# WilliamYi96/HGR-Net

Measured on AMD Instinct MI355X. Metric: images/sec over 21K-class hierarchy, batch 512; hit@1 parity vs reference, higher is better.
Workload: dtype f16

## Files before the change

hgr-net_amd/_lib.py:

```python
from __future__ import annotations

import ctypes as C
import os
from pathlib import Path

import torch

_HERE = Path(__file__).resolve().parent
LIB_PATH = Path(os.environ.get("HGR_LIB", _HERE / "lib" / "libhgr.so"))

HGR_BF16, HGR_F16 = 0, 1
EPI_NONE, EPI_BIAS, EPI_BIAS_QUICKGELU, EPI_BIAS_RESIDUAL, EPI_BIAS_RELU, EPI_BIAS_ADD16_RELU, EPI_ACCUM, EPI_QGELU_GRAD16 = 0, 1, 2, 3, 4, 5, 6, 7

_p, _i, _l, _f = C.c_void_p, C.c_int, C.c_int64, C.c_float

SIGNATURES = {
    "hgr_gemm_nt": [_p, _l, _p, _l, _p, _l, _p, _p, _l, _i, _i, _i, _i, _i, _i, _p],
    "hgr_gemm_set_tile": [_i],
    "hgr_gemm_set_tail": [_i, _i],
    "hgr_gemm_set_persist": [_i],
    "hgr_gemm_set_ws": [_i],
    "hgr_gemm_set_p8": [_i],
    "hgr_im2col_patches": [_p, _p, _i, _i, _i, _i, _i, _p],
    "hgr_im2col_patches_ex": [_p, _p, _i, _i, _i, _i, _i, _i, _i, _p],
# ... 41 lines not shown
    "hgr_ctx_splice_bwd": [_p, _p, _i, _i, _i, _i, _p],
    "hgr_sumsq": [_p, _l, _p, _p],
    "hgr_eval_counters": [_p, _i, _p, _i, _p, _p, _i, _p, _p, _i, _p, _i, _p],
    "hgr_eval_counters_rows": [_p, _i, _p, _p, _p, _i, _p, _p, _p, _i, _p, _i, _p],
    "hgr_eval_report_rows": [_p, _i, _p, _p, _p, _i, _p, _p, _p, _i, _p, _i, _p],
    "hgr_path_scores": [_p, _l, _p, _l, _i, _p, _p, _p, _i, _p],
    "hgr_subtree_hedge": [_p, _l, _i, _p, _p, _p, _f, _p, _i, _p, _p, _p, _l, _i, _p],
    "hgr_hedge_counters_rows": [_p, _i, _p, _p, _p, _i, _p, _i, _p],
    "hgr_set_ranks": [_p, _l, _i, _p, _p, _i, _p, _p, _p, _i, _p],
    "hgr_set_counters_rows": [_p, _p, _i, _p, _p, _i, _p, _p, _p, _i, _p, _i, _p],
    "hgr_dot_f32":[_p, _p, _l, _p, _f, _i, _p],
    "hgr_conv3x3_nhwc_plain": [_p, _p, _p, _i, _i, _i, _i, _i, _i, _i, _p],
    "hgr_gemm_nt_splitk": [_p, _l, _p, _l, _p, _l, _i, _i, _i, _i, _i, _p],
    "hgr_gemm_tn_splitk": [_p, _l, _p, _l, _p, _l, _i, _i, _i, _i, _i, _p],
    "hgr_gemm_tn_tile": [_i, _i],
    "hgr_gemm_plan_capture": [_p, _i],
    "hgr_conv3x3_wgrad_splitk": [_p, _l, _p, _p, _l, _i, _i, _i, _i, _i, _i, _i, _p],
    "hgr_relu_bwd16": [_p, _p, _p, _l, _i, _p],
    "hgr_add16": [_p, _p, _p, _l, _i, _p],
    "hgr_avgpool2_bwd_nhwc": [_p, _p, _i, _i, _i, _i, _i, _p],
    "hgr_attnpool_tokens_bwd": [_p, _p, _i, _i, _i, _i, _p],
    "hgr_im2col3x3_t": [_p, _p, _i, _i, _i, _i, _l, _i, _p],
    "hgr_bn_fold": [_p, _p, _p, _p, _p, _f, _p, _p, _i, _i, _i, _i, _i, _p],
    "hgr_bn_unfold_grad": [_p, _l, _p, _p, _p, _p, _p, _f, _p, _p, _p, _i, _i, _i, _p],
    "hgr_csr_group_aggregate": [_p, _l, _p, _p, _p, _p, _i, _p, _p, _p, _p, _i, _p, _p, _p, _p, _i, _p, _p, _l, _i, _f, _i, _p],
    "hgr_gemm_nt_res_stats": [_p, _l, _p, _l, _p, _p, _l, _p, _p, _i, _i, _i, _i, _p],
    "hgr_vit_head": [_p, _p, _l, _l, _p, _p, _f, _p, _p, _i, _i, _i, _i, _p],
    "hgr_gemm_nt_res_stats_guard": [_p, _l, _p, _l, _p, _p, _l, _p, _p, _f, _p, _i, _i, _i, _i, _p],
    "hgr_gemm_nt_ln": [_p, _l, _p, _l, _p, _l, _p, _p, _p, _f, _i, _i, _i, _i, _i, _p],
    "hgr_gemm_nt_ln_mha": [_p, _l, _p, _l, _p, _p, _p, _f, _p, _l, _i, _i, _i, _i, _i, _p],
    "hgr_gemm_nt_bias_gelu_dual": [_p, _l, _p, _l, _p, _l, _p, _l, _p, _i, _i, _i, _i, _p],
    "hgr_gemm_nt_qgelu_grad_colsum": [_p, _l, _p, _l, _p, _l, _p, _l, _p, _i, _i, _i, _i, _p],
    "hgr_vit_embed_ln_stats": [_p, _p, _p, _p, _p, _p, _p, _p, _i, _i, _i, _f, _i, _p],
    "hgr_row_stats16": [_p, _p, _p, _p, _i, _i, _i, _p],
    "hgr_pair_rows_f32": [_p, _p, _p, _i, _i, _l, _p, _i, _p],
    "hgr_logits_eval_workspace_bytes": [_i, _i],
    "hgr_logits_eval": [_p, _p, _i, _i, _i, _p, _p, _p, _i, _p, _p, _i, _p, _i, _i, _p, _p, _p, _p, _i, _p],
    "hgr_logits_eval_tile_stage": [_p, _p, _i, _i, _i, _p, _p, _p, _i, _p, _p, _i, _p, _i, _i, _p, _p, _p, _p, _i, _p],
    "hgr_logits_eval_row_stage": [_p, _p, _i, _i, _i, _p, _p, _p, _i, _p, _p, _i, _p, _i, _i, _p, _p, _p, _p, _i, _p],
    "hgr_comm_unique_id": [_p],
    "hgr_comm_init": [_i, _i, _p],
    "hgr_comm_destroy": [],
    "hgr_comm_rank": [],
    "hgr_comm_world": [],
    "hgr_allreduce": [_p, _p, _l, _i, _i, _p],
    "hgr_allgather": [_p, _p, _l, _i, _p],
    "hgr_broadcast": [_p, _l, _i, _i, _p],
    "hgr_adamw": [_p, _p, _p, _p, _l, _f, _f, _f, _f, _f, _i, _p, _f, _f, _p],
}


class GemmLaunch(C.Structure):
    _fields_ = [(name, C.c_int32) for name in ("kernel", "variant", "epilogue", "out_f32", "act", "grid_x", "grid_y", "tiles_m", "tiles_n", "total",
                                                "nbig", "big_panels", "tiles_m_half", "group", "m_fastest", "vec_ok", "row0", "rows")]


class HgrError(RuntimeError):
    pass


_lib = None


ABI_VERSION = 5


# ... 43 lines not shown
```

hgr-net_amd/clip/model.py:

```python
from __future__ import annotations

import os
from collections import OrderedDict
from typing import Dict, Optional, Tuple, Union

import numpy as np
import torch
from torch import nn

from .. import ops
from .._lib import (EPI_BIAS, EPI_BIAS_ADD16_RELU, EPI_BIAS_QUICKGELU, EPI_BIAS_RELU, EPI_BIAS_RESIDUAL, EPI_NONE,
                    HgrError)


class QuickGELU(nn.Module):
    """Placeholder so ``mlp`` keeps the reference's child names (c_fc, gelu, c_proj); the activation
    itself is fused into the c_fc GEMM epilogue (HGR_EPI_BIAS_QUICKGELU)."""


class ResidualAttentionBlock(nn.Module):
    def __init__(self, d_model: int, n_head: int):
        super().__init__()
        self.attn = nn.MultiheadAttention(d_model, n_head)
        self.ln_1 = nn.LayerNorm(d_model)
# ... 99 lines not shown
        w32, g32, be32 = w.detach().float(), ln.weight.detach().float(), ln.bias.detach().float()
        wf = (w32 * g32[None, :]).to(dt).contiguous()
        return wf, wf.float().sum(dim=1).contiguous(), (w32 @ be32 + b.detach().float()).contiguous()


class _Workspace:

    def __init__(self):
        self._b: Dict[str, torch.Tensor] = {}
        self.epoch = 0

    def const(self, name: str, build) -> torch.Tensor:
        t = self._b.get("const." + name)
        if t is None:
            t = self._b["const." + name] = build()
            self.epoch += 1
        return t

    def get(self, name: str, shape, dtype, device) -> torch.Tensor:
        n = int(np.prod(shape))
        t = self._b.get(name)
        if t is None or t.numel() < n or t.dtype != dtype or t.device != device:
            t = torch.empty(n, dtype=dtype, device=device)
            self._b[name] = t
            self.epoch += 1
        return t[:n].view(*shape)


IMG_STREAMS = max(1, int(os.environ.get("HGR_IMG_STREAMS", "1")))
IMG_STREAMS_MIN_ROWS = 8192
CLS_LAST = os.environ.get("HGR_CLS_LAST", "1") != "0"
LN_FUSED = os.environ.get("HGR_LN_FUSED", "1") != "0"
QKV_MHA = os.environ.get("HGR_QKV_MHA", "1") != "0"


def ln_fusable(w: int, m: int = 0) -> bool:
    return LN_FUSED and w % 128 == 0 and m * 4 * w * 2 < 2 ** 32


def _run_blocks(x: Optional[torch.Tensor], blocks, heads: int, b: int, l: int, causal: bool, dt: torch.dtype, ws: _Workspace, tag: str,
                taps: Optional[dict] = None, tap_prefix: str = "", pair=None, stats: Optional[torch.Tensor] = None,
                flag: Optional[torch.Tensor] = None, cls_only_last: bool = False):
    m, w = (pair[0] if pair is not None else x).shape
    dev = (pair[0] if pair is not None else x).device
    qkv = ws.get(tag + ".qkv", (m, 3 * w), dt, dev)
    att = ws.get(tag + ".att", (m, w), dt, dev)
    u16 = ws.get(tag + ".u16", (m, 4 * w), dt, dev)
    if pair is not None:
        xh, xl = pair
        for i, k in enumerate(blocks):
            last_cls = cls_only_last and i == len(blocks) - 1 and l > 1 and 3 * w * l < (1 << 23)
            fused_attn = QKV_MHA and not last_cls and ops.ln_mha_ok(w, l, m, xh.stride(0))
            if last_cls:
                ch, cl = xh.view(b, l, w)[:, 0, :], xl.view(b, l, w)[:, 0, :]
                ops.gemm_nt_ln(xh, k.wf_in[w:], qkv[:, w:], k.s_in[w:], k.c_in[w:], stats, k.eps1, tag="kv")
                ops.split_point("class_token_tail")
                st_q = ws.get(tag + ".stats_q", (b, w // 64, 2), torch.float32, dev)
                idx = ws.const(f"cls_rows.{b}.{l}", lambda: (torch.arange(b, dtype=torch.int32, device=dev) * l).contiguous())
                ops.rows_gather(stats.view(b * l, -1), idx, st_q.view(b, -1))
                ops.gemm_nt_ln(ch, k.wf_in[:w], qkv.view(b, l, 3 * w)[:, 0, :w], k.s_in[:w], k.c_in[:w], st_q, k.eps1, tag="q_cls")
            elif fused_attn:
                ops.gemm_nt_ln_mha(xh, k.wf_in, att, k.s_in, k.c_in, stats, b, l, heads, causal, k.eps1)
            else:
                ops.gemm_nt_ln(xh, k.wf_in, qkv, k.s_in, k.c_in, stats, k.eps1, tag="qkv")
            if not fused_attn:
                ops.mha(qkv, att, b, l, heads, causal, q_rows=1 if last_cls else 0)
# ... 285 lines not shown
            fused = self._vit_forward(image, p, out, tag, taps, u8)
            if fused and self._ln_check("v", dev):
                self._vit_forward(image, p, out, tag, taps, u8)
            return out
        main = torch.cuda.current_stream()
        side = self._side_streams(ns - 1, dev)
        cut = [b * i // ns for i in range(ns + 1)]
        fused = False
        for i in range(ns):
            st = main if i == 0 else side[i - 1]
            if i:
                st.wait_stream(main)
            with torch.cuda.stream(st):
                fused |= self._vit_forward(image[cut[i]:cut[i + 1]], p, out[cut[i]:cut[i + 1]], f"v{i}" if i else "v", None, u8)
        for st in side:
            main.wait_stream(st)
        if fused and self._ln_check("v", dev):
            self._vit_forward(image, p, out, "v", None, u8)
        return out

    def _side_streams(self, n: int, dev):
        have = self.__dict__.setdefault("_streams", [])
        while len(have) < n:
            have.append(torch.cuda.Stream(device=dev))
        return have[:n]

    def _vit_forward(self, image: torch.Tensor, p: dict, out: torch.Tensor, tag: str, taps: Optional[dict], u8: bool) -> bool:
        v = self.visual
        dt, ws, dev = self.image_dtype, self._ws, image.device
        b, r = image.shape[0], v.input_resolution
        ps = v.patch_size
        g = r // ps
        gg, l, w = g * g, g * g + 1, v.conv1.weight.shape[0]
        patches = ws.get(tag + ".patches", (b * gg, p["kp"]), dt, dev)
        if u8:
            ops.im2col_patches_u8(image, patches, ps)
        else:
            ops.im2col_patches(image, patches, ps)
        pe = ws.get(tag + ".pe", (b * gg, w), torch.float32, dev)
        ops.gemm_nt(patches, p["conv_w_nhwc"] if u8 else p["conv_w"], pe, tag="patch")
        cls16 = ws.get(tag + ".cls16", (b, w), dt, dev)
        fused = ln_fusable(w, b * l) and "v" not in self._ln_off
        if fused:
            xh = ws.get(tag + ".xh", (b * l, w), dt, dev)
            xl = ws.get(tag + ".xl", (b * l, w), ops.PAIR_LO, dev)
            stats = ws.get(tag + ".stats", (b * l, w // 64, 2), torch.float32, dev)
            ops.vit_embed_ln_stats(pe, p["cls"], p["pos"], p["ln_pre"][0], p["ln_pre"][1], xh, xl, stats, b, gg)
            if taps is not None:
                taps["visual.ln_pre"] = ops.pair_value(xh, xl).view(b, l, w)
            _run_blocks(None, p["vblocks"], w // 64, b, l, False, dt, ws, tag, taps, "visual.transformer", (xh, xl), stats, self._ln_flag("v", dev),
                        cls_only_last=taps is None and CLS_LAST)
            if w <= 1920 and w % 32 == 0 and v.output_dim % 4 == 0:
                ops.vit_head(xh, xl, l, p["ln_post"][0], p["ln_post"][1], float(v.ln_post.eps), p["proj_t"], out)
                return fused
            cls32 = ws.get(tag + ".cls32", (b, w), torch.float32, dev)
            ops.pair_rows_f32(xh, xl, cls32, row_mul=l)
            ops.layernorm(cls32, p["ln_post"][0], p["ln_post"][1], cls16, rows=b)
        else:
            x = ws.get(tag + ".x", (b * l, w), torch.float32, dev)
            ops.vit_embed_ln(pe, p["cls"], p["pos"], p["ln_pre"][0], p["ln_pre"][1], x, b, gg)
            if taps is not None:
                taps["visual.ln_pre"] = x.view(b, l, w).clone()
            _run_blocks(x, p["vblocks"], w // 64, b, l, False, dt, ws, tag, taps, "visual.transformer")
            ops.layernorm(x, p["ln_post"][0], p["ln_post"][1], cls16, rows=b, row_mul=l)
        ops.gemm_nt(cls16, p["proj_t"], out)
        return fused

    @torch.no_grad()
    def encode_text(self, text: torch.Tensor, trim: bool = True, ctx: Optional[torch.Tensor] = None) -> torch.Tensor:
        if not text.is_cuda:
            raise HgrError("encode_text needs a device tensor: the product path has no CPU fallback")
        p = self._prepared()
        dt, ws, dev = self.text_dtype, self._ws, text.device
        text = text.long()
        n, ctx_len = text.shape
        w = self.transformer.width
        d = self.text_projection.shape[1]
        out = torch.empty((n, d), dtype=torch.float32, device=dev)
        eot = torch.empty(n, dtype=torch.int32, device=dev)
        ops.eot_index(text, eot)
# ... 68 lines not shown
```

hgr-net_amd/csrc/hgr_common.h:

```cpp
#pragma once
#include <hip/hip_runtime.h>
#include <stdint.h>
#include <stdio.h>
#include <stdarg.h>
#include <stdlib.h>
#include <type_traits>

#include "../../include/hgr.h"

#define HGR_WAVE 64

#ifdef HGR_LAB
#define HGR_LAB_ON(expr) (expr)
static inline int hgr_lab_env(const char *name) { const char *e = getenv(name); return e ? atoi(e) : 0; }
#else
#define HGR_LAB_ON(expr) false
static inline int hgr_lab_env(const char *) { return 0; }
#endif

typedef __attribute__((ext_vector_type(8))) __bf16 bf16x8;
typedef __attribute__((ext_vector_type(8))) _Float16 f16x8;
typedef __attribute__((ext_vector_type(4))) __bf16 bf16x4;
typedef __attribute__((ext_vector_type(4))) _Float16 f16x4;
typedef __attribute__((ext_vector_type(4))) float f32x4;
// ... 128 lines not shown
__device__ __forceinline__ float wave_max(float v) {
#pragma unroll
    for (int o = 32; o > 0; o >>= 1) v = fmaxf(v, __shfl_xor(v, o));
    return v;
}
__device__ __forceinline__ unsigned long long wave_max_u64(unsigned long long v) {
#pragma unroll
    for (int o = 32; o > 0; o >>= 1) {
        const unsigned lo = __shfl_xor((unsigned)v, o), hi = __shfl_xor((unsigned)(v >> 32), o);
        const unsigned long long w = ((unsigned long long)hi << 32) | lo;
        v = w > v ? w : v;
    }
    return v;
}

__device__ __forceinline__ unsigned orderable(float v) { const unsigned u = __float_as_uint(v); return u ^ ((u >> 31) ? 0xFFFFFFFFu : 0x80000000u); }
__device__ __forceinline__ float unorderable(unsigned u) { return __uint_as_float(u ^ ((u >> 31) ? 0x80000000u : 0xFFFFFFFFu)); }
__device__ __forceinline__ unsigned long long key_of(float v, int p) { return ((unsigned long long)orderable(v) << 32) | (unsigned)(0x7fffffff - p); }
__device__ __forceinline__ void key_decode(unsigned long long m, float &v, int &p) { v = unorderable((unsigned)(m >> 32)); p = 0x7fffffff - (int)(unsigned)m; }

__device__ __forceinline__ int level_pick(const int32_t *__restrict__ lv_row, int n_levels, int le) {
    return (unsigned)le < (unsigned)n_levels ? lv_row[le] : -2;
}
__device__ __forceinline__ unsigned path_edges(unsigned mm, int L) { return L == 1 ? (mm & 1u) : (unsigned)__popc(mm & (mm >> 1)); }

__device__ __forceinline__ float row16_sum(float v) {
    v += __builtin_bit_cast(float, __builtin_amdgcn_update_dpp(0, __builtin_bit_cast(int, v), 0xB1, 0xF, 0xF, true));
    v += __builtin_bit_cast(float, __builtin_amdgcn_update_dpp(0, __builtin_bit_cast(int, v), 0x4E, 0xF, 0xF, true));
    v += __builtin_bit_cast(float, __builtin_amdgcn_update_dpp(0, __builtin_bit_cast(int, v), 0x141, 0xF, 0xF, true));
    v += __builtin_bit_cast(float, __builtin_amdgcn_update_dpp(0, __builtin_bit_cast(int, v), 0x140, 0xF, 0xF, true));
    return v;
}

int hgr_set_error(int code, const char *fmt, ...);

#define HGR_REQUIRE(cond, ...)                                            \
    do {                                                                  \
        if (!(cond)) return hgr_set_error(HGR_EINVAL, __VA_ARGS__);       \
    } while (0)

#define HGR_CHECK_LAUNCH(name)                                                                      \
    do {                                                                                            \
        hipError_t e__ = hipGetLastError();                                                         \
        if (e__ != hipSuccess) return hgr_set_error(HGR_ELAUNCH, "%s: %s", name, hipGetErrorString(e__)); \
    } while (0)

static inline bool hgr_aligned(const void *p, size_t a) { return (reinterpret_cast<uintptr_t>(p) % a) == 0; }

int hgr_cu_count();

template <typename T = int> struct HgrKnob {
    const char *env; T def; T (*clamp)(T) = nullptr;
    bool known = false; T v = T();
    T get() {
        if (!known) {
            const char *e = getenv(env);
            v = !e ? def : std::is_floating_point<T>::value ? (T)atof(e) : (T)atoi(e);
            if (clamp) v = clamp(v);
            known = true;
        }
        return v;
    }
    T set(T nv) { const T prev = get(); v = nv; return prev; }
};
static inline int hgr_knob_bool(int v) { return v != 0; }
```

hgr-net_amd/csrc/hgr_norm.hip:

```cpp
#include "hgr_common.h"

namespace {

constexpr int MAXV = 16;

template <int DT, bool OUT32, int NV>
__global__ __launch_bounds__(256) void layernorm_rows(const float *__restrict__ x, const float *__restrict__ gamma,
                                                      const float *__restrict__ beta, void *__restrict__ y,
                                                      int rows, int W, int64_t row_mul, const int32_t *__restrict__ row_idx, float eps) {
    const int lane = threadIdx.x & 63;
    const int row = blockIdx.x * 4 + (threadIdx.x >> 6);
    if (row >= rows) return;
    const int64_t src = (int64_t)row * row_mul + (row_idx ? row_idx[row] : 0);
    const f32x4 *xr = (const f32x4 *)(x + src * W);
    const int nv = W >> 2;
    f32x4 v[NV];
    float s = 0.f;
#pragma unroll
    for (int i = 0; i < NV; ++i) {
        const int c = i * 64 + lane;
        if (i * 64 < nv) {
            v[i] = (c < nv) ? xr[c] : (f32x4){0.f, 0.f, 0.f, 0.f};
            s += v[i][0] + v[i][1] + v[i][2] + v[i][3];
        }
// ... 18 lines not shown
            f32x4 o;
#pragma unroll
            for (int e = 0; e < 4; ++e) o[e] = (v[i][e] - mean) * rstd * ga[e] + be[e];
            if (OUT32) ((f32x4 *)((float *)y + (int64_t)row * W))[c] = o;
            else ((typename T16<DT>::vec4 *)((typename T16<DT>::elem *)y + (int64_t)row * W))[c] = cvt4<DT>(o[0], o[1], o[2], o[3]);
        }
    }
}

template <int NV, int DT = HGR_F16, bool STATS = false>
__global__ __launch_bounds__(256) void vit_embed_ln(const float *__restrict__ patches, const float *__restrict__ cls,
                                                    const float *__restrict__ pos, const float *__restrict__ gamma,
                                                    const float *__restrict__ beta, float *__restrict__ x,
                                                    int B, int G, int W, float eps, void *__restrict__ xh = nullptr, void *__restrict__ xl = nullptr,
                                                    float *__restrict__ stats = nullptr) {
    const int lane = threadIdx.x & 63;
    const int L = G + 1;
    const int row = blockIdx.x * 4 + (threadIdx.x >> 6);
    if (row >= B * L) return;
    const int b = row / L, t = row - b * L;
    const f32x4 *src = (const f32x4 *)(t == 0 ? cls : patches + ((int64_t)b * G + (t - 1)) * W);
    const f32x4 *pr = (const f32x4 *)(pos + (int64_t)t * W);
    const int nv = W >> 2;
    f32x4 v[NV];
    float s = 0.f;
#pragma unroll
    for (int i = 0; i < NV; ++i) {
        const int c = i * 64 + lane;
        if (i * 64 < nv) {
            v[i] = (c < nv) ? (src[c] + pr[c]) : (f32x4){0.f, 0.f, 0.f, 0.f};
            s += v[i][0] + v[i][1] + v[i][2] + v[i][3];
        }
    }
    const float mean = wave_sum(s) / (float)W;
    float q = 0.f;
#pragma unroll
    for (int i = 0; i < NV; ++i) {
        const int c = i * 64 + lane;
        if (i * 64 < nv && c < nv) {
#pragma unroll
            for (int e = 0; e < 4; ++e) { const float d = v[i][e] - mean; q += d * d; }
        }
    }
    const float rstd = rsqrtf(wave_sum(q) / (float)W + eps);
    const f32x4 *gv = (const f32x4 *)gamma, *bv = (const f32x4 *)beta;
    f32x4 *out = STATS ? nullptr : (f32x4 *)(x + (int64_t)row * W);
#pragma unroll
    for (int i = 0; i < NV; ++i) {
        const int c = i * 64 + lane;
        if (i * 64 < nv && c < nv) {
            const f32x4 ga = gv[c], be = bv[c];
            f32x4 o;
#pragma unroll
            for (int e = 0; e < 4; ++e) o[e] = (v[i][e] - mean) * rstd * ga[e] + be[e];
            if (!STATS) out[c] = o;
            if (STATS) {
                typename T16<DT>::vec4 nh;
                unsigned nl = 0u;
#pragma unroll
                for (int e = 0; e < 4; ++e) { unsigned q; typename T16<DT>::elem h; pair_split<DT>(o[e], h, q); nh[e] = h; nl |= q << (8 * e); }
                ((typename T16<DT>::vec4 *)((typename T16<DT>::elem *)xh + (int64_t)row * W))[c] = nh;
                ((unsigned *)((unsigned char *)xl + (int64_t)row * W))[c] = nl;
                const float s1 = row16_sum((o[0] + o[1]) + (o[2] + o[3]));
                const float s2 = row16_sum((o[0] * o[0] + o[1] * o[1]) + (o[2] * o[2] + o[3] * o[3]));
                if ((lane & 15) == 0) *(float2 *)(stats + ((int64_t)row * (W >> 6) + (c >> 4)) * 2) = make_float2(s1, s2);
            }
        }
    }
}

template <int DT>
__global__ __launch_bounds__(256) void row_stats16(const float *__restrict__ x, void *__restrict__ xh, void *__restrict__ xl, float *__restrict__ stats, int rows, int W) {
    const int lane = threadIdx.x & 63;
    const int row = blockIdx.x * 4 + (threadIdx.x >> 6);
    if (row >= rows) return;
    const f32x4 *xr = (const f32x4 *)(x + (int64_t)row * W);
    const int nv = W >> 2;
    for (int c0 = 0; c0 < nv; c0 += 64) {
        const int c = c0 + lane;
        const bool ok = c < nv;
        const f32x4 v = ok ? xr[c] : (f32x4){0.f, 0.f, 0.f, 0.f};
        const float s1 = row16_sum((v[0] + v[1]) + (v[2] + v[3]));
        const float s2 = row16_sum((v[0] * v[0] + v[1] * v[1]) + (v[2] * v[2] + v[3] * v[3]));
        if (ok) {
            typename T16<DT>::vec4 nh;
            unsigned nl = 0u;
#pragma unroll
            for (int e = 0; e < 4; ++e) { unsigned q; typename T16<DT>::elem h; pair_split<DT>(v[e], h, q); nh[e] = h; nl |= q << (8 * e); }
            ((typename T16<DT>::vec4 *)((typename T16<DT>::elem *)xh + (int64_t)row * W))[c] = nh;
            ((unsigned *)((unsigned char *)xl + (int64_t)row * W))[c] = nl;
            if ((lane & 15) == 0) *(float2 *)(stats + ((int64_t)row * (W >> 6) + (c >> 4)) * 2) = make_float2(s1, s2);
        }
    }
}

template <int DT>
__global__ __launch_bounds__(256) void pair_rows_f32(const void *__restrict__ xh, const void *__restrict__ xl, float *__restrict__ out, int rows, int W,
                                                     int64_t row_mul, const int32_t *__restrict__ row_idx) {
    const int lane = threadIdx.x & 63;
    const int row = blockIdx.x * 4 + (threadIdx.x >> 6);
    if (row >= rows) return;
// ... 253 lines not shown
```

hgr-net_amd/ops.py:

```python
from __future__ import annotations

import math
from typing import Optional

import torch

from . import _lib
from ._lib import (EPI_ACCUM, EPI_BIAS, EPI_BIAS_ADD16_RELU, EPI_BIAS_QUICKGELU, EPI_BIAS_RELU, EPI_BIAS_RESIDUAL, EPI_NONE, EPI_QGELU_GRAD16,
                   HGR_BF16, HGR_F16)

PROFILE = None

WEIGHTS_GEN = [0]

SPLIT_HOOK = None


def split_point(name: str) -> None:
    h = SPLIT_HOOK
    if h is not None:
        h(name)


TORCH16 = {HGR_BF16: torch.bfloat16, HGR_F16: torch.float16}
# ... 114 lines not shown
    assert x16.stride(1) == wfold.stride(1) == out.stride(1) == 1 and stats.dtype == torch.float32 and stats.numel() >= m * (k // 64) * 2
    ev = _prof_begin()
    _lib.call("hgr_gemm_nt_ln", _dev(x16), x16.stride(0), _dev(wfold), wfold.stride(0), _dev(out), out.stride(0), _dev(ln_s), _dev(ln_c),
              _dev(stats), float(eps), m, n, k, DT_OF[x16.dtype], 1 if quickgelu else 0, _stream())
    _prof_end(ev, 2.0 * m * n * k, 2 * m * k + 2 * n * k + 2 * m * n, tag)
    return out


def gemm_nt_ln_mha(x16: torch.Tensor, wfold: torch.Tensor, att: torch.Tensor, ln_s: torch.Tensor, ln_c: torch.Tensor, stats: torch.Tensor,
                   b: int, l: int, heads: int, causal: bool, eps: float = 1e-5, tag: str = "qkv_mha") -> torch.Tensor:
    m, k = x16.shape
    w = heads * 64
    assert m == b * l and k == w and wfold.shape == (3 * w, k) and x16.dtype == wfold.dtype == att.dtype and att.shape == (m, w)
    assert x16.stride(1) == wfold.stride(1) == att.stride(1) == 1 and ln_s.numel() == ln_c.numel() == 3 * w
    assert stats.dtype == torch.float32 and stats.numel() >= m * (k // 64) * 2
    ev = _prof_begin()
    _lib.call("hgr_gemm_nt_ln_mha", _dev(x16), x16.stride(0), _dev(wfold), wfold.stride(0), _dev(ln_s), _dev(ln_c), _dev(stats), float(eps),
              _dev(att), att.stride(0), b, l, heads, 1 if causal else 0, DT_OF[x16.dtype], _stream())
    _prof_end(ev, 2.0 * m * 3 * w * k + 4.0 * b * heads * l * l * 64, 2 * m * k + 2 * 3 * w * k + 2 * m * w, tag)
    return att


def ln_mha_ok(w: int, l: int, rows: Optional[int] = None, ldx: Optional[int] = None) -> bool:
    if not (1 <= l <= 64 and w % 128 == 0):
        return False
    if rows is not None and rows * (ldx if ldx is not None else w) * 2 >= (1 << 32):
        return False
    return 3 * w * w * 2 < (1 << 32)


def vit_embed_ln_stats(patches, cls, pos, gamma, beta, xh, xl, stats, b, g, eps=1e-5):
    _lib.call("hgr_vit_embed_ln_stats", _dev(patches), _dev(cls), _dev(pos), _dev(gamma), _dev(beta), _dev(xh), _dev(xl), _dev(stats),
              b, g, xh.shape[1], eps, DT_OF[xh.dtype], _stream())


def row_stats16(x: torch.Tensor, xh: torch.Tensor, xl: torch.Tensor, stats: torch.Tensor) -> None:
    assert x.dtype == torch.float32 and x.is_contiguous() and xh.is_contiguous() and xl.is_contiguous() and xh.shape == xl.shape == x.shape
    assert xl.dtype == PAIR_LO and stats.numel() >= x.shape[0] * (x.shape[1] // 64) * 2
    _lib.call("hgr_row_stats16", _dev(x), _dev(xh), _dev(xl), _dev(stats), x.shape[0], x.shape[1], DT_OF[xh.dtype], _stream())


def pair_rows_f32(xh: torch.Tensor, xl: torch.Tensor, out: torch.Tensor, row_mul: int = 1, row_idx: Optional[torch.Tensor] = None) -> torch.Tensor:
    assert xh.is_contiguous() and xl.is_contiguous() and out.is_contiguous() and out.dtype == torch.float32 and out.shape[1] == xh.shape[1] and xl.dtype == PAIR_LO
    _lib.call("hgr_pair_rows_f32", _dev(xh), _dev(xl), _dev(out), out.shape[0], out.shape[1], row_mul, _dev(row_idx), DT_OF[xh.dtype], _stream())
    return out


def vit_head(xh: torch.Tensor, xl: torch.Tensor, row_mul: int, gamma: torch.Tensor, beta: torch.Tensor, eps: float, proj_t: torch.Tensor,
             out: torch.Tensor) -> torch.Tensor:
    assert xh.dtype == proj_t.dtype and xl.dtype == PAIR_LO and xh.stride() == xl.stride() and xh.stride(1) == 1
    assert out.dtype == torch.float32 and out.is_contiguous() and proj_t.is_contiguous() and proj_t.shape[1] == xh.shape[1] and out.shape[1] == proj_t.shape[0]
    ev = _prof_begin()
    _lib.call("hgr_vit_head", _dev(xh), _dev(xl), xh.stride(0), int(row_mul), _dev(gamma), _dev(beta), float(eps), _dev(proj_t), _dev(out),
              out.shape[0], xh.shape[1], out.shape[1], DT_OF[xh.dtype], _stream())
    _prof_end(ev, 2.0 * out.shape[0] * out.shape[1] * xh.shape[1], 0, "head")
    return out


def gemm_set_tile(tile: int) -> int:
    lib = _lib.load()
    prev = lib.hgr_gemm_set_tile(int(tile))
    if prev < 0:
        raise _lib.HgrError(f"hgr_gemm_set_tile failed ({prev}): {lib.hgr_last_error().decode()}")
    return prev


# ... 784 lines not shown
```

include/hgr.h:

```cpp
#ifndef HGR_H
#define HGR_H

#include <stdint.h>

#ifdef __cplusplus
extern "C" {
#endif

#define HGR_ABI_VERSION 5

enum { HGR_OK = 0, HGR_EINVAL = -1, HGR_EUNSUPPORTED = -2, HGR_ELAUNCH = -3 };

typedef enum { HGR_BF16 = 0, HGR_F16 = 1 } hgr_dtype_t;

typedef enum {
    HGR_EPI_NONE = 0,
    HGR_EPI_BIAS = 1,
    HGR_EPI_BIAS_QUICKGELU = 2,
    HGR_EPI_BIAS_RESIDUAL = 3,
    HGR_EPI_BIAS_RELU = 4,
    HGR_EPI_BIAS_ADD16_RELU = 5,
    HGR_EPI_ACCUM = 6,
    HGR_EPI_QGELU_GRAD16 = 7
} hgr_epilogue_t;
// ... 205 lines not shown
int hgr_ctx_splice_bwd(float *dx, float *dctx, int n, int L, int W, int n_ctx, void *stream);

int hgr_rows_gather(float *dst, const float *src, const int32_t *idx, int rows, int W, void *stream);

int hgr_sumsq(const float *x, int64_t n, float *out, void *stream);

int hgr_adamw(float *p, const float *g, float *m, float *v, int64_t n, float lr, float beta1, float beta2, float eps,
              float wd, int step, const float *sumsq_total, float max_norm, float grad_scale, void *stream);

int hgr_gemm_nt_res_stats(const void *A, int64_t lda, const void *W, int64_t ldw, void *xh, void *xl, int64_t ldx,
                          const float *bias, float *stats, int M, int N, int K, int dtype, void *stream);

int hgr_gemm_nt_res_stats_guard(const void *A, int64_t lda, const void *W, int64_t ldw, void *xh, void *xl, int64_t ldx,
                                const float *bias, float *stats, float guard_sumsq, uint32_t *flag,
                                int M, int N, int K, int dtype, void *stream);

int hgr_vit_head(const void *xh, const void *xl, int64_t ldx, int64_t row_mul, const float *gamma, const float *beta, float eps,
                 const void *proj_t, float *out, int B, int W, int D, int dtype, void *stream);
int hgr_gemm_nt_ln(const void *XH, int64_t ldx, const void *Wfold, int64_t ldw, void *C, int64_t ldc,
                   const float *ln_s, const float *ln_c, const float *stats, float eps,
                   int M, int N, int K, int dtype, int act, void *stream);

int hgr_gemm_nt_ln_mha(const void *XH, int64_t ldx, const void *Wfold, int64_t ldw, const float *ln_s, const float *ln_c,
                       const float *stats, float eps, void *att, int64_t ldatt, int B, int L, int heads, int causal,
                       int dtype, void *stream);

int hgr_gemm_nt_bias_gelu_dual(const void *A, int64_t lda, const void *W, int64_t ldw, void *pre, int64_t ldpre, void *post, int64_t ldpost,
                               const float *bias, int M, int N, int K, int dtype, void *stream);
int hgr_gemm_nt_qgelu_grad_colsum(const void *A, int64_t lda, const void *W, int64_t ldw, void *C, int64_t ldc, const void *pre, int64_t ldpre,
                                  float *colsum_part, int M, int N, int K, int dtype, void *stream);
int hgr_vit_embed_ln_stats(const float *patches, const float *class_embedding, const float *positional_embedding,
                           const float *gamma, const float *beta, void *xh, void *xl, float *stats,
                           int B, int G, int W, float eps, int dtype, void *stream);
int hgr_row_stats16(const float *x, void *xh, void *xl, float *stats, int rows, int W, int dtype, void *stream);
int hgr_pair_rows_f32(const void *xh, const void *xl, float *out, int rows, int W, int64_t row_mul, const int32_t *row_idx, int dtype, void *stream);

int64_t hgr_logits_eval_workspace_bytes(int rows, int n_perm);
int hgr_logits_eval(const void *feat16, const void *zsl_perm16, int rows, int D, int n_perm,
                    const int32_t *tpos_perm, const int32_t *epos_perm, const int32_t *level_first,
                    int n_levels, const int32_t *filler_pos, const int32_t *train_cols, int n_train,
                    const int32_t *test_cols, int n_test, int k,
                    int32_t *out_level, int32_t *out_top1, int32_t *out_topk, void *workspace, int dtype, void *stream);
int hgr_logits_eval_tile_stage(const void *feat16, const void *zsl_perm16, int rows, int D, int n_perm,
                    const int32_t *tpos_perm, const int32_t *epos_perm, const int32_t *level_first,
                    int n_levels, const int32_t *filler_pos, const int32_t *train_cols, int n_train,
                    const int32_t *test_cols, int n_test, int k,
                    int32_t *out_level, int32_t *out_top1, int32_t *out_topk, void *workspace, int dtype, void *stream);
int hgr_logits_eval_row_stage(const void *feat16, const void *zsl_perm16, int rows, int D, int n_perm,
                    const int32_t *tpos_perm, const int32_t *epos_perm, const int32_t *level_first,
                    int n_levels, const int32_t *filler_pos, const int32_t *train_cols, int n_train,
                    const int32_t *test_cols, int n_test, int k,
                    int32_t *out_level, int32_t *out_top1, int32_t *out_topk, void *workspace, int dtype, void *stream);

#define HGR_COMM_ID_BYTES 128
typedef enum { HGR_COMM_F32 = 0, HGR_COMM_F64 = 1, HGR_COMM_F16 = 2, HGR_COMM_BF16 = 3, HGR_COMM_I32 = 4, HGR_COMM_I64 = 5, HGR_COMM_U8 = 6 } hgr_comm_dtype_t;
typedef enum { HGR_COMM_SUM = 0, HGR_COMM_MAX = 1 } hgr_comm_op_t;

int hgr_comm_unique_id(void *id_out );
int hgr_comm_init(int rank, int world, const void *unique_id );
int hgr_comm_destroy(void);
int hgr_comm_rank(void);
int hgr_comm_world(void);
int hgr_allreduce(const void *send, void *recv, int64_t count, int dtype, int op, void *stream);
int hgr_allgather(const void *send, void *recv, int64_t count_per_rank, int dtype, void *stream);
int hgr_broadcast(void *buf, int64_t count, int dtype, int root, void *stream);

// ... 5 lines not shown
```

Baseline: 106,400.

## Fuse ViT patch im2col, patch GEMM and ln_pre into one kernel

Adds a single kernel that DMAs raw f32 image patches and conv weights into LDS, runs the patch-embedding GEMM with MFMA for two images per block, then adds positional and class embeddings and applies ln_pre with pair split and stats in the epilogue. It replaces the separate im2col, GEMM to an f32 buffer and embed+LN passes, removing the intermediate patches and pe round trips through global memory. It is limited to ViT-B/32-like shapes (P=32, W=768, at most 56 patches per image) and f32 contiguous non-u8 input. Its grid is only (B+1)/2 blocks with converted-on-the-fly A fragments, so occupancy and GEMM efficiency may be lower than the general GEMM.

```diff
diff --git a/hgr-net_amd/_lib.py b/hgr-net_amd/_lib.py
--- a/hgr-net_amd/_lib.py
+++ b/hgr-net_amd/_lib.py
@@ -97,6 +97,8 @@
     "hgr_gemm_nt_bias_gelu_dual": [_p, _l, _p, _l, _p, _l, _p, _l, _p, _i, _i, _i, _i, _p],
     "hgr_gemm_nt_qgelu_grad_colsum": [_p, _l, _p, _l, _p, _l, _p, _l, _p, _i, _i, _i, _i, _p],
     "hgr_vit_embed_ln_stats": [_p, _p, _p, _p, _p, _p, _p, _p, _i, _i, _i, _f, _i, _p],
+    "hgr_vit_patch_embed_ln_ok": [_i, _i, _i, _i, _i],
+    "hgr_vit_patch_embed_ln": [_p, _p, _p, _p, _p, _p, _p, _p, _p, _i, _i, _i, _i, _f, _i, _p],
     "hgr_row_stats16": [_p, _p, _p, _p, _i, _i, _i, _p],
     "hgr_pair_rows_f32": [_p, _p, _p, _i, _i, _l, _p, _i, _p],
     "hgr_logits_eval_workspace_bytes": [_i, _i],
diff --git a/hgr-net_amd/clip/model.py b/hgr-net_amd/clip/model.py
--- a/hgr-net_amd/clip/model.py
+++ b/hgr-net_amd/clip/model.py
@@ -155,6 +155,7 @@
 CLS_LAST = os.environ.get("HGR_CLS_LAST", "1") != "0"
 LN_FUSED = os.environ.get("HGR_LN_FUSED", "1") != "0"
 QKV_MHA = os.environ.get("HGR_QKV_MHA", "1") != "0"
+PATCH_FUSED = os.environ.get("HGR_PATCH_FUSED", "1") != "0"
 
 
 def ln_fusable(w: int, m: int = 0) -> bool:
@@ -506,20 +507,26 @@
         ps = v.patch_size
         g = r // ps
         gg, l, w = g * g, g * g + 1, v.conv1.weight.shape[0]
-        patches = ws.get(tag + ".patches", (b * gg, p["kp"]), dt, dev)
-        if u8:
-            ops.im2col_patches_u8(image, patches, ps)
-        else:
-            ops.im2col_patches(image, patches, ps)
-        pe = ws.get(tag + ".pe", (b * gg, w), torch.float32, dev)
-        ops.gemm_nt(patches, p["conv_w_nhwc"] if u8 else p["conv_w"], pe, tag="patch")
+        fused = ln_fusable(w, b * l) and "v" not in self._ln_off
+        one_launch = (PATCH_FUSED and fused and not u8 and image.dtype == torch.float32 and image.is_contiguous() and p["kp"] == 3 * ps * ps
+                      and ops.vit_patch_embed_ln_ok(b, r, ps, w, dt))
+        if not one_launch:
+            patches = ws.get(tag + ".patches", (b * gg, p["kp"]), dt, dev)
+            if u8:
+                ops.im2col_patches_u8(image, patches, ps)
+            else:
+                ops.im2col_patches(image, patches, ps)
+            pe = ws.get(tag + ".pe", (b * gg, w), torch.float32, dev)
+            ops.gemm_nt(patches, p["conv_w_nhwc"] if u8 else p["conv_w"], pe, tag="patch")
         cls16 = ws.get(tag + ".cls16", (b, w), dt, dev)
-        fused = ln_fusable(w, b * l) and "v" not in self._ln_off
         if fused:
             xh = ws.get(tag + ".xh", (b * l, w), dt, dev)
             xl = ws.get(tag + ".xl", (b * l, w), ops.PAIR_LO, dev)
             stats = ws.get(tag + ".stats", (b * l, w // 64, 2), torch.float32, dev)
-            ops.vit_embed_ln_stats(pe, p["cls"], p["pos"], p["ln_pre"][0], p["ln_pre"][1], xh, xl, stats, b, gg)
+            if one_launch:
+                ops.vit_patch_embed_ln(image, p["conv_w"], p["cls"], p["pos"], p["ln_pre"][0], p["ln_pre"][1], xh, xl, stats, ps)
+            else:
+                ops.vit_embed_ln_stats(pe, p["cls"], p["pos"], p["ln_pre"][0], p["ln_pre"][1], xh, xl, stats, b, gg)
             if taps is not None:
                 taps["visual.ln_pre"] = ops.pair_value(xh, xl).view(b, l, w)
             _run_blocks(None, p["vblocks"], w // 64, b, l, False, dt, ws, tag, taps, "visual.transformer", (xh, xl), stats, self._ln_flag("v", dev),
diff --git a/hgr-net_amd/csrc/hgr_common.h b/hgr-net_amd/csrc/hgr_common.h
--- a/hgr-net_amd/csrc/hgr_common.h
+++ b/hgr-net_amd/csrc/hgr_common.h
@@ -184,6 +184,48 @@
     return v;
 }
 
+#define HGR_VIT_LN_ROW_BODY \
+    const float mean = wave_sum(s) / (float)W; \
+    float q = 0.f; \
+_Pragma("unroll") \
+    for (int i = 0; i < NV; ++i) { \
+        const int c = i * 64 + lane; \
+        if (i * 64 < nv && c < nv) { \
+_Pragma("unroll") \
+            for (int e = 0; e < 4; ++e) { const float d = v[i][e] - mean; q += d * d; } \
+        } \
+    } \
+    const float rstd = rsqrtf(wave_sum(q) / (float)W + eps); \
+    const f32x4 *gv = (const f32x4 *)gamma, *bv = (const f32x4 *)beta; \
+    f32x4 *out = STATS ? nullptr : (f32x4 *)(x + (int64_t)row * W); \
+_Pragma("unroll") \
+    for (int i = 0; i < NV; ++i) { \
+        const int c = i * 64 + lane; \
+        if (i * 64 < nv && c < nv) { \
+            const f32x4 ga = gv[c], be = bv[c]; \
+            f32x4 o; \
+_Pragma("unroll") \
+            for (int e = 0; e < 4; ++e) o[e] = (v[i][e] - mean) * rstd * ga[e] + be[e]; \
+            if (!STATS) out[c] = o; \
+            if (STATS) { \
+                typename T16<DT>::vec4 nh; \
+                unsigned nl = 0u; \
+_Pragma("unroll") \
+                for (int e = 0; e < 4; ++e) { unsigned q; typename T16<DT>::elem h; pair_split<DT>(o[e], h, q); nh[e] = h; nl |= q << (8 * e); } \
+                ((typename T16<DT>::vec4 *)((typename T16<DT>::elem *)xh + (int64_t)row * W))[c] = nh; \
+                ((unsigned *)((unsigned char *)xl + (int64_t)row * W))[c] = nl; \
+                const float s1 = row16_sum((o[0] + o[1]) + (o[2] + o[3])); \
+                const float s2 = row16_sum((o[0] * o[0] + o[1] * o[1]) + (o[2] * o[2] + o[3] * o[3])); \
+                if ((lane & 15) == 0) *(float2 *)(stats + ((int64_t)row * (W >> 6) + (c >> 4)) * 2) = make_float2(s1, s2); \
+            } \
+        } \
+    }
+template <int NV, int DT, bool STATS>
+__device__ __forceinline__ void vit_ln_row(const f32x4 (&v)[NV], float s, int lane, int nv, int W, float eps, const float *gamma, const float *beta,
+                                           float *x, int row, void *xh, void *xl, float *stats) {
+    HGR_VIT_LN_ROW_BODY
+}
+
 int hgr_set_error(int code, const char *fmt, ...);
 
 #define HGR_REQUIRE(cond, ...)                                            \
diff --git a/hgr-net_amd/csrc/hgr_norm.hip b/hgr-net_amd/csrc/hgr_norm.hip
--- a/hgr-net_amd/csrc/hgr_norm.hip
+++ b/hgr-net_amd/csrc/hgr_norm.hip
@@ -74,41 +74,7 @@
             s += v[i][0] + v[i][1] + v[i][2] + v[i][3];
         }
     }
-    const float mean = wave_sum(s) / (float)W;
-    float q = 0.f;
-#pragma unroll
-    for (int i = 0; i < NV; ++i) {
-        const int c = i * 64 + lane;
-        if (i * 64 < nv && c < nv) {
-#pragma unroll
-            for (int e = 0; e < 4; ++e) { const float d = v[i][e] - mean; q += d * d; }
-        }
-    }
-    const float rstd = rsqrtf(wave_sum(q) / (float)W + eps);
-    const f32x4 *gv = (const f32x4 *)gamma, *bv = (const f32x4 *)beta;
-    f32x4 *out = STATS ? nullptr : (f32x4 *)(x + (int64_t)row * W);
-#pragma unroll
-    for (int i = 0; i < NV; ++i) {
-        const int c = i * 64 + lane;
-        if (i * 64 < nv && c < nv) {
-            const f32x4 ga = gv[c], be = bv[c];
-            f32x4 o;
-#pragma unroll
-            for (int e = 0; e < 4; ++e) o[e] = (v[i][e] - mean) * rstd * ga[e] + be[e];
-            if (!STATS) out[c] = o;
-            if (STATS) {
-                typename T16<DT>::vec4 nh;
-                unsigned nl = 0u;
-#pragma unroll
-                for (int e = 0; e < 4; ++e) { unsigned q; typename T16<DT>::elem h; pair_split<DT>(o[e], h, q); nh[e] = h; nl |= q << (8 * e); }
-                ((typename T16<DT>::vec4 *)((typename T16<DT>::elem *)xh + (int64_t)row * W))[c] = nh;
-                ((unsigned *)((unsigned char *)xl + (int64_t)row * W))[c] = nl;
-                const float s1 = row16_sum((o[0] + o[1]) + (o[2] + o[3]));
-                const float s2 = row16_sum((o[0] * o[0] + o[1] * o[1]) + (o[2] * o[2] + o[3] * o[3]));
-                if ((lane & 15) == 0) *(float2 *)(stats + ((int64_t)row * (W >> 6) + (c >> 4)) * 2) = make_float2(s1, s2);
-            }
-        }
-    }
+    HGR_VIT_LN_ROW_BODY
 }
 
 template <int DT>
diff --git a/hgr-net_amd/csrc/hgr_patch_embed.hip b/hgr-net_amd/csrc/hgr_patch_embed.hip
--- /dev/null
+++ b/hgr-net_amd/csrc/hgr_patch_embed.hip
@@ -0,0 +1,215 @@
+#include "hgr_gemm_common.h"
+
+namespace hgr_gemm {
+namespace {
+constexpr int PE_NT = 512;
+constexpr int PE_W = 768, PE_P = 32, PE_K = 3 * PE_P * PE_P, PE_NK = PE_K / 32;
+constexpr int PE_MT = 7, PE_ROWS = 16 * PE_MT;
+constexpr int PE_A = 0, PE_W0 = 32768, PE_W1 = 81920;
+constexpr int PE_ASZ = 16384, PE_WSZ = 24576;
+constexpr int PE_RS = PE_W * 4 + 16, PE_PR = 48;
+constexpr int PE_LDS = PE_PR * PE_RS;
+static_assert(PE_W1 + 2 * PE_WSZ <= PE_LDS, "the stages fit under the epilogue's rows");
+
+template <int DT>
+__global__ __launch_bounds__(PE_NT) void vit_patch_embed_ln(const float *__restrict__ image, const char *__restrict__ conv_w, const float *__restrict__ cls,
+                                                            const float *__restrict__ pos, const float *__restrict__ gamma, const float *__restrict__ beta,
+                                                            void *__restrict__ xh, void *__restrict__ xl, float *__restrict__ stats,
+                                                            int B, int R, int gs, float eps) {
+    typedef typename T16<DT>::vec8 vec8;
+    typedef typename T16<DT>::elem E;
+    __shared__ __attribute__((aligned(1024))) char smem[PE_LDS];
+
+    const int tid = threadIdx.x;
+    const int lane = tid & 63;
+    const int wave = __builtin_amdgcn_readfirstlane(tid >> 6);
+    const int grp = wave >> 2;
+    const int r = lane & 15, g = lane >> 4;
+    const int gg = gs * gs;
+    const int img0 = blockIdx.x * 2;
+    const bool two = img0 + 1 < B;
+    const int64_t img_elems = (int64_t)3 * R * R;
+    const char *const abase = (const char *)(image + (int64_t)img0 * img_elems);
+
+    unsigned oA[2], oW[3];
+#pragma unroll
+    for (int i = 0; i < 3; ++i) {
+        const int id = (i * 8 + wave) * 64 + lane;
+        const int line = id >> 3, slot = id & 7;
+        if (i < 2) {
+            const int pr = line;
+            const int c = ((((slot >> 1) ^ ((pr >> 1) & 3)) << 1) | ((slot & 1) ^ (((pr + 4) >> 3) & 1)));
+            int tr = pr < 2 * gg ? pr : 0;
+            const int im = tr >= gg ? 1 : 0;
+            const int patch = tr - im * gg;
+            const int gy = patch / gs, gx = patch - gy * gs;
+            oA[i] = (unsigned)((((int64_t)((im && two) ? 1 : 0) * img_elems + (int64_t)gy * PE_P * R + gx * PE_P) * 4) + c * 16);
+        }
+        const int c8 = slot ^ (line & 7);
+        const int q = 2 * line + (c8 >> 2);
+        const int n = 96 * (q / 48) + q % 48;
+        oW[i] = (unsigned)(n * (PE_K * 2) + (c8 & 3) * 16);
+    }
+    char *const ldsw = smem + wave * 1024;
+    const __amdgpu_buffer_rsrc_t rA = dma_rsrc(abase), rW = dma_rsrc(conv_w);
+    const int RR4 = R * R * 4, R4 = R * 4;
+    auto issueA = [&](int t) {
+        char *dst = ldsw + PE_A + (t & 1) * PE_ASZ;
+        const int ts = min(t, PE_NK - 1);
+        const int soff = (ts >> 5) * RR4 + (ts & 31) * R4;
+#pragma unroll
+        for (int i = 0; i < 2; ++i) dma16(rA, abase, oA[i], soff, dst + i * 8192);
+    };
+    auto issueW = [&](int half, int t) {
+        char *dst = ldsw + (half ? PE_W1 : PE_W0) + (t & 1) * PE_WSZ;
+#pragma unroll
+        for (int i = 0; i < 3; ++i) dma16(rW, conv_w, oW[i], min(t, PE_NK - 1) * 64 + half * (48 * PE_K * 2), dst + i * 8192);
+    };
+
+    const int offA = r * 128 + ((g ^ ((r >> 1) & 3)) << 5);
+    const int hsA = (((r + 4) >> 3) & 1) << 4;
+    const int offW = (24 * wave + (r >> 1)) * 128 + ((((r & 1) * 4 + g) ^ (r >> 1)) << 4);
+
+    f32x4 acc[PE_MT][6];
+#pragma unroll
+    for (int i = 0; i < PE_MT; ++i)
+#pragma unroll
+        for (int j = 0; j < 6; ++j) acc[i][j] = (f32x4){0.f, 0.f, 0.f, 0.f};
+    vec8 af[PE_MT], wf[3];
+
+    issueA(0); issueW(0, 0);
+    issueW(1, 0);
+    issueA(1); issueW(0, 1);
+    HGR_RWAIT(8);
+    if (grp) HGR_MBAR();
+
+    for (int t = 0; t < PE_NK; ++t) {
+        const char *sa = smem + PE_A + (t & 1) * PE_ASZ, *sw0 = smem + PE_W0 + (t & 1) * PE_WSZ, *sw1 = smem + PE_W1 + (t & 1) * PE_WSZ;
+#pragma unroll
+        for (int j = 0; j < 3; ++j) wf[j] = *(const vec8 *)(sw0 + offW + j * 1024);
+#pragma unroll
+        for (int i = 0; i < PE_MT; ++i) {
+            const f32x4 lo = *(const f32x4 *)(sa + offA + i * 2048 + hsA);
+            const f32x4 hi = *(const f32x4 *)(sa + offA + i * 2048 + (16 - hsA));
+            vec8 a;
+            a[0] = (E)lo[0]; a[1] = (E)lo[1]; a[2] = (E)lo[2]; a[3] = (E)lo[3];
+            a[4] = (E)hi[0]; a[5] = (E)hi[1]; a[6] = (E)hi[2]; a[7] = (E)hi[3];
+            af[i] = a;
+        }
+        issueW(1, t + 1);
+        HGR_RWAIT(8);
+        __builtin_amdgcn_s_setprio(1);
+#pragma unroll
+        for (int i = 0; i < PE_MT; ++i)
+#pragma unroll
+            for (int j = 0; j < 3; ++j) acc[i][j] = T16<DT>::mfma16(wf[j], af[i], acc[i][j]);
+        __builtin_amdgcn_s_setprio(0);
+        HGR_MBAR();
+#pragma unroll
+        for (int j = 0; j < 3; ++j) wf[j] = *(const vec8 *)(sw1 + offW + j * 1024);
+        issueA(t + 2); issueW(0, t + 2);
+        HGR_RWAIT(8);
+        __builtin_amdgcn_s_setprio(1);
+#pragma unroll
+        for (int i = 0; i < PE_MT; ++i)
+#pragma unroll
+            for (int j = 0; j < 3; ++j) acc[i][3 + j] = T16<DT>::mfma16(wf[j], af[i], acc[i][3 + j]);
+        __builtin_amdgcn_s_setprio(0);
+        HGR_MBAR();
+    }
+    if (!grp) HGR_MBAR();
+    asm volatile("s_waitcnt vmcnt(0)" ::: "memory");
+
+    const int L = gg + 1;
+    constexpr int nv = PE_W >> 2;
+    int tid_e = threadIdx.x;
+    asm volatile("" : "+v"(tid_e));
+    const int lane_e = tid_e & 63, r_e = lane_e & 15, g_e = lane_e >> 4;
+#pragma unroll
+    for (int pass = 0; pass < 3; ++pass) {
+        __syncthreads();
+        if (pass * PE_PR < 2 * gg) {
+#pragma unroll
+            for (int ii = 0; ii < 3; ++ii) {
+                const int i = pass * 3 + ii;
+                if (i < PE_MT) {
+#pragma unroll
+                    for (int j = 0; j < 6; ++j)
+                        *(f32x4 *)(smem + (ii * 16 + r_e) * PE_RS + (96 * wave + 16 * j + 4 * g_e) * 4) = acc[i < PE_MT ? i : 0][j];
+                }
+            }
+        }
+        __syncthreads();
+        int ln = lane_e;
+        asm volatile("" : "+v"(ln));
+#pragma unroll
+        for (int k = 0; k < PE_PR / 8; ++k) {
+            const int lr = k * 8 + wave, tr = pass * PE_PR + lr;
+            const int im = tr >= gg ? 1 : 0;
+            if (tr < 2 * gg && tr < PE_ROWS && (!im || two)) {
+                const int patch = tr - im * gg;
+                const f32x4 *src = (const f32x4 *)(smem + lr * PE_RS), *pr = (const f32x4 *)(pos + (int64_t)(1 + patch) * PE_W);
+                f32x4 v[4];
+                float s = 0.f;
+#pragma unroll
+                for (int i = 0; i < 4; ++i) {
+                    const int c = i * 64 + ln;
+                    if (i * 64 < nv) {
+                        v[i] = (c < nv) ? (src[c] + pr[c]) : (f32x4){0.f, 0.f, 0.f, 0.f};
+                        s += v[i][0] + v[i][1] + v[i][2] + v[i][3];
+                    }
+                }
+                vit_ln_row<4, DT, true>(v, s, ln, nv, PE_W, eps, gamma, beta, nullptr, (img0 + im) * L + 1 + patch, xh, xl, stats);
+            }
+        }
+    }
+
+    if (wave < 2 && (wave == 0 || two)) {
+        const f32x4 *src = (const f32x4 *)cls, *pr = (const f32x4 *)pos;
+        f32x4 v[4];
+        float s = 0.f;
+#pragma unroll
+        for (int i = 0; i < 4; ++i) {
+            const int c = i * 64 + lane_e;
+            if (i * 64 < nv) {
+                v[i] = (c < nv) ? (src[c] + pr[c]) : (f32x4){0.f, 0.f, 0.f, 0.f};
+                s += v[i][0] + v[i][1] + v[i][2] + v[i][3];
+            }
+        }
+        vit_ln_row<4, DT, true>(v, s, lane_e, nv, PE_W, eps, gamma, beta, nullptr, (img0 + wave) * L, xh, xl, stats);
+    }
+}
+
+}
+}
+
+extern "C" int hgr_vit_patch_embed_ln_ok(int B, int R, int P, int W, int dtype) {
+    if (B < 1 || P != hgr_gemm::PE_P || R < P || R % P != 0 || W != hgr_gemm::PE_W) return 0;
+    const int gs = R / P;
+    if (gs * gs > hgr_gemm::PE_ROWS / 2) return 0;
+    if ((int64_t)B * (gs * gs + 1) >= (int64_t)1 << 31) return 0;
+    return dtype == HGR_BF16 || dtype == HGR_F16;
+}
+
+extern "C" int hgr_vit_patch_embed_ln(const float *image, const void *conv_w, const float *class_embedding, const float *positional_embedding,
+                                      const float *gamma, const float *beta, void *xh, void *xl, float *stats,
+                                      int B, int R, int P, int W, float eps, int dtype, void *stream) {
+    using namespace hgr_gemm;
+    HGR_REQUIRE(image && conv_w && class_embedding && positional_embedding && gamma && beta && xh && xl && stats, "hgr_vit_patch_embed_ln: null operand");
+    HGR_REQUIRE(dtype == HGR_BF16 || dtype == HGR_F16, "hgr_vit_patch_embed_ln: bad dtype %d", dtype);
+    HGR_REQUIRE(P == PE_P, "hgr_vit_patch_embed_ln: patch size P=%d unsupported (32)", P);
+    HGR_REQUIRE(W == PE_W, "hgr_vit_patch_embed_ln: width W=%d unsupported (768)", W);
+    HGR_REQUIRE(B >= 1 && R >= P && R % P == 0, "hgr_vit_patch_embed_ln: B=%d R=%d unsupported (R a multiple of %d)", B, R, P);
+    const int gs = R / P, gg = gs * gs;
+    HGR_REQUIRE(gg <= PE_ROWS / 2, "hgr_vit_patch_embed_ln: %d patches per image exceed %d (two images per 112-row tile)", gg, PE_ROWS / 2);
+    HGR_REQUIRE((int64_t)B * (gg + 1) < ((int64_t)1 << 31), "hgr_vit_patch_embed_ln: B=%d: %lld rows exceed 32-bit row indices", B, (long long)B * (gg + 1));
+    HGR_REQUIRE((int64_t)2 * 3 * R * R * 4 < ((int64_t)1 << 31) && (int64_t)PE_W * PE_K * 2 < ((int64_t)1 << 31), "hgr_vit_patch_embed_ln: operand offsets exceed 32 bits");
+    HGR_REQUIRE(hgr_aligned(image, 16) && hgr_aligned(conv_w, 16) && hgr_aligned(class_embedding, 16) && hgr_aligned(positional_embedding, 16) &&
+                hgr_aligned(gamma, 16) && hgr_aligned(beta, 16) && hgr_aligned(xh, 16) && hgr_aligned(xl, 16) && hgr_aligned(stats, 16),
+                "hgr_vit_patch_embed_ln: operands must be 16-byte aligned");
+    const dim3 grid((B + 1) / 2), block(PE_NT);
+    if (dtype == HGR_BF16) hipLaunchKernelGGL((vit_patch_embed_ln<HGR_BF16>), grid, block, 0, (hipStream_t)stream, image, (const char *)conv_w, class_embedding, positional_embedding, gamma, beta, xh, xl, stats, B, R, gs, eps);
+    else hipLaunchKernelGGL((vit_patch_embed_ln<HGR_F16>), grid, block, 0, (hipStream_t)stream, image, (const char *)conv_w, class_embedding, positional_embedding, gamma, beta, xh, xl, stats, B, R, gs, eps);
+    HGR_CHECK_LAUNCH("hgr_vit_patch_embed_ln");
+    return HGR_OK;
+}
diff --git a/hgr-net_amd/ops.py b/hgr-net_amd/ops.py
--- a/hgr-net_amd/ops.py
+++ b/hgr-net_amd/ops.py
@@ -170,6 +170,26 @@
 def vit_embed_ln_stats(patches, cls, pos, gamma, beta, xh, xl, stats, b, g, eps=1e-5):
     _lib.call("hgr_vit_embed_ln_stats", _dev(patches), _dev(cls), _dev(pos), _dev(gamma), _dev(beta), _dev(xh), _dev(xl), _dev(stats),
               b, g, xh.shape[1], eps, DT_OF[xh.dtype], _stream())
+
+
+def vit_patch_embed_ln_ok(b: int, r: int, patch: int, w: int, dtype) -> bool:
+    code = DT_OF.get(dtype, dtype if isinstance(dtype, int) else -1)
+    return bool(_lib.load().hgr_vit_patch_embed_ln_ok(int(b), int(r), int(patch), int(w), int(code)))
+
+
+def vit_patch_embed_ln(image: torch.Tensor, conv_w: torch.Tensor, cls, pos, gamma, beta, xh, xl, stats, patch: int, eps=1e-5) -> None:
+    assert image.dtype == torch.float32 and image.dim() == 4 and image.shape[1] == 3 and image.shape[2] == image.shape[3] and image.is_contiguous()
+    b, r = image.shape[0], image.shape[2]
+    w, k = conv_w.shape
+    gg = (r // patch) ** 2
+    assert conv_w.is_contiguous() and k == 3 * patch * patch and conv_w.dtype == xh.dtype and xl.dtype == PAIR_LO
+    assert xh.is_contiguous() and xl.is_contiguous() and xh.shape == xl.shape == (b * (gg + 1), w)
+    assert stats.dtype == torch.float32 and stats.is_contiguous() and stats.numel() >= b * (gg + 1) * (w // 64) * 2
+    ev = _prof_begin()
+    _lib.call("hgr_vit_patch_embed_ln", _dev(image), _dev(conv_w), _dev(cls), _dev(pos), _dev(gamma), _dev(beta), _dev(xh), _dev(xl), _dev(stats),
+              b, r, patch, w, eps, DT_OF[xh.dtype], _stream())
+    rows = b * (gg + 1)
+    _prof_end(ev, 2.0 * b * gg * w * k, 4 * b * 3 * r * r + 2 * w * k + 3 * rows * w + 8 * rows * (w // 64), "patch")
 
 
 def row_stats16(x: torch.Tensor, xh: torch.Tensor, xl: torch.Tensor, stats: torch.Tensor) -> None:
diff --git a/include/hgr.h b/include/hgr.h
--- a/include/hgr.h
+++ b/include/hgr.h
@@ -261,6 +261,10 @@
 int hgr_vit_embed_ln_stats(const float *patches, const float *class_embedding, const float *positional_embedding,
                            const float *gamma, const float *beta, void *xh, void *xl, float *stats,
                            int B, int G, int W, float eps, int dtype, void *stream);
+int hgr_vit_patch_embed_ln_ok(int B, int R, int P, int W, int dtype);
+int hgr_vit_patch_embed_ln(const float *image, const void *conv_w, const float *class_embedding, const float *positional_embedding,
+                           const float *gamma, const float *beta, void *xh, void *xl, float *stats,
+                           int B, int R, int P, int W, float eps, int dtype, void *stream);
 int hgr_row_stats16(const float *x, void *xh, void *xl, float *stats, int rows, int W, int dtype, void *stream);
 int hgr_pair_rows_f32(const void *xh, const void *xl, float *out, int rows, int W, int64_t row_mul, const int32_t *row_idx, int dtype, void *stream);
 
```

New measurement: 107,800 (median of 6 runs). 1.3% higher.
